# amoretti86/PSVO

Hardware: AMD Instinct MI355X
Metric: particle-steps/sec (higher is better)
Workload: dtype f32

## Files before the change

### psvo_amd/csrc/common.h

```cpp
#pragma once
#include <cstddef>
#include <type_traits>
#include <hip/hip_runtime.h>
#include <stdint.h>

#include "../../include/psvo_hip.h"

#ifndef PSVO_L
#define PSVO_L 1
#endif
#if PSVO_L == 1
#define PSVO_LNS l1
#define PSVO_ENTRY(name) extern "C" int name
#define PSVO_L2_DECL(name) extern "C" __attribute__((visibility("hidden"))) decltype(name) name##_l2;
#elif PSVO_L == 2
#define PSVO_LNS l2
#define PSVO_ENTRY(name) extern "C" __attribute__((visibility("hidden"))) int name##_l2
#define PSVO_L2_DECL(name)
#else
#error "PSVO_L must be 1 or 2"
#endif

namespace psvo {

// ... 434 lines not shown
#pragma unroll
            for (int o = 0; o < DOUT; ++o) gr[o] = lane_fetch(dout[o], src);
            float pre1[NQ][4];
            layer1(w, g, xr, pre1);
            f4v D[NQ];
            hidden2(w, g, r, pre1, D);
            float dp[NQ][4];
#pragma unroll
            for (int jt = 0; jt < NQ; ++jt) {
                float s[4] = {0.f, 0.f, 0.f, 0.f};
#pragma unroll
                for (int o = 0; o < DOUT; ++o) {
                    const float4 wo = *reinterpret_cast<const float4*>(w + kW2 + o * H + 16 * jt + 4 * g);
                    s[0] = fmaf(gr[o], wo.x, s[0]); s[1] = fmaf(gr[o], wo.y, s[1]);
                    s[2] = fmaf(gr[o], wo.z, s[2]); s[3] = fmaf(gr[o], wo.w, s[3]);
                }
#pragma unroll
                for (int v = 0; v < 4; ++v) dp[jt][v] = D[jt][v] > 0.f ? s[v] : 0.f;
            }
            f4v E[NQ];
#pragma unroll
            for (int kt = 0; kt < NQ; ++kt) E[kt] = f4v{0.f, 0.f, 0.f, 0.f};
            const float* wb = w + kWh + 4 * g * kWS + r;
#pragma unroll
            for (int jt = 0; jt < NQ; ++jt) {
#pragma unroll
                for (int v = 0; v < 4; ++v) {
#pragma unroll
                    for (int kt = 0; kt < NQ; ++kt) {
                        const float a = wb[(16 * jt + v) * kWS + 16 * kt];
                        E[kt] = __builtin_amdgcn_mfma_f32_16x16x4f32(a, dp[jt][v], E[kt], 0, 0, 0);
                    }
                }
            }
            float acc[DIN];
#pragma unroll
            for (int d = 0; d < DIN; ++d) acc[d] = 0.f;
#pragma unroll
            for (int q = 0; q < NQ; ++q) {
                float e[4];
#pragma unroll
                for (int c = 0; c < 4; ++c) e[c] = pre1[q][c] > 0.f ? E[q][c] : 0.f;
#pragma unroll
                for (int d = 0; d < DIN; ++d) {
                    const float4 wi = *reinterpret_cast<const float4*>(w + kW1 + d * H + 16 * q + 4 * g);
                    acc[d] = fmaf(e[0], wi.x, fmaf(e[1], wi.y, fmaf(e[2], wi.z, fmaf(e[3], wi.w, acc[d]))));
                }
            }
#pragma unroll
            for (int d = 0; d < DIN; ++d) {
                float v = acc[d];
                v += xor_lane<16>(v);
                v += xor_lane<32>(v);
                const float t = lane_fetch(v, my_row & 15);
                if (mine && (my_row >> 4) == p) dx[d] += t;
            }
        }
    }

    template <bool ROLLED = false>
    __device__ __forceinline__ static void eval(const float* __restrict__ w, const float (&x)[DIN], float (&out)[DOUT]) {
        eval_rows<1, 0>(w, true, x, out);
    }
    template <int S, int PB = 0>
    __device__ __forceinline__ static void eval_part(const float* __restrict__ w, int , const float (&x)[DIN],
                                                     float (&out)[DOUT]) {
        eval_rows<S, PB>(w, true, x, out);
    }
    template <bool ROLLED = false>
    __device__ __forceinline__ static void bwd_input(const float* __restrict__ w, const float (&x)[DIN],
                                                     const float (&dout)[DOUT], float (&dx)[DIN]) {
        bwd_rows<1, 0>(w, x, dout, dx);
    }
    template <int S, int PB = 0>
    __device__ __forceinline__ static void bwd_input_part(const float* __restrict__ w, int , const float (&x)[DIN],
                                                          const float (&dout)[DOUT], float (&dx)[DIN]) {
        bwd_rows<S, PB>(w, x, dout, dx);
    }
};
#endif

template <int D>
__device__ __forceinline__ float diag_lp(const float (&x)[D], const float (&mu)[D], const float (&inv_s)[D],
                                         float cst) {
    float acc = 0.f;
#pragma unroll
    for (int d = 0; d < D; ++d) {
        const float z = (x[d] - mu[d]) * inv_s[d];
        acc = fmaf(z, z, acc);
    }
    return fmaf(-0.5f, acc, cst);
}

template <int CTRL, int ROW_MASK = 0xF, int BANK_MASK = 0xF, bool BOUND = false>
__device__ __forceinline__ float dpp_mov(float old, float v) {
    return __builtin_bit_cast(float, __builtin_amdgcn_update_dpp(__builtin_bit_cast(int, old), __builtin_bit_cast(int, v),
                                                                  CTRL, ROW_MASK, BANK_MASK, BOUND));
}

template <int MASK>
__device__ __forceinline__ float xor_lane(float v) {
    static_assert(MASK == 1 || MASK == 2 || MASK == 4 || MASK == 8 || MASK == 16 || MASK == 32, "xor_lane mask");
    if constexpr (MASK == 1) {
        return dpp_mov<0xB1, 0xF, 0xF, true>(v, v);
    } else if constexpr (MASK == 2) {
        return dpp_mov<0x4E, 0xF, 0xF, true>(v, v);
    } else if constexpr (MASK == 4) {
        float t = dpp_mov<0x104, 0xF, 0x5>(v, v);
        return dpp_mov<0x114, 0xF, 0xA>(t, v);
    } else if constexpr (MASK == 8) {
        return dpp_mov<0x128, 0xF, 0xF, true>(v, v);
    } else if constexpr (MASK == 16) {
        const unsigned u = __builtin_bit_cast(unsigned, v);
        const auto p = __builtin_amdgcn_permlane16_swap(u, u, false, false);
        const bool odd_row = (__lane_id() >> 4) & 1;
        return __builtin_bit_cast(float, odd_row ? p[0] : p[1]);
    } else {
        const unsigned u = __builtin_bit_cast(unsigned, v);
        const auto p = __builtin_amdgcn_permlane32_swap(u, u, false, false);
        return __builtin_bit_cast(float, (__lane_id() >= 32) ? p[0] : p[1]);
    }
}

__device__ __forceinline__ float wave_incl_scan(float v, int ) {
    v += dpp_mov<0x111, 0xF, 0xF, true>(0.f, v);
    v += dpp_mov<0x112, 0xF, 0xF, true>(0.f, v);
    v += dpp_mov<0x114, 0xF, 0xF, true>(0.f, v);
    v += dpp_mov<0x118, 0xF, 0xF, true>(0.f, v);
    v += dpp_mov<0x142, 0xA, 0xF, false>(0.f, v);
    v += dpp_mov<0x143, 0xC, 0xF, false>(0.f, v);
    return v;
}
__device__ __forceinline__ float wave_sum(float v) {
    v = wave_incl_scan(v, 0);
    return __builtin_bit_cast(float, __builtin_amdgcn_readlane(__builtin_bit_cast(int, v), 63));
}
__device__ __forceinline__ float wave_max(float v) {
    const float ninf = -__builtin_huge_valf();
    v = fmaxf(v, dpp_mov<0x111>(ninf, v));
    v = fmaxf(v, dpp_mov<0x112>(ninf, v));
    v = fmaxf(v, dpp_mov<0x114>(ninf, v));
    v = fmaxf(v, dpp_mov<0x118>(ninf, v));
    v = fmaxf(v, dpp_mov<0x142, 0xA>(ninf, v));
    v = fmaxf(v, dpp_mov<0x143, 0xC>(ninf, v));
    return __builtin_bit_cast(float, __builtin_amdgcn_readlane(__builtin_bit_cast(int, v), 63));
}
__device__ __forceinline__ void quad_bcast4(float v, float (&out)[4]) {
    out[0] = dpp_mov<0x00>(v, v);
    out[1] = dpp_mov<0x55>(v, v);
    out[2] = dpp_mov<0xAA>(v, v);
    out[3] = dpp_mov<0xFF>(v, v);
}

template <int G>
__device__ __forceinline__ float group_sum(float v) {
    if constexpr (G > 1) v += xor_lane<1>(v);
    if constexpr (G > 2) v += xor_lane<2>(v);
    if constexpr (G > 4) v += xor_lane<4>(v);
    if constexpr (G > 8) v += xor_lane<8>(v);
    if constexpr (G > 16) v += xor_lane<16>(v);
    if constexpr (G > 32) v += xor_lane<32>(v);
    return v;
}
template <int G>
__device__ __forceinline__ float group_max(float v) {
    if constexpr (G > 1) v = fmaxf(v, xor_lane<1>(v));
    if constexpr (G > 2) v = fmaxf(v, xor_lane<2>(v));
    if constexpr (G > 4) v = fmaxf(v, xor_lane<4>(v));
    if constexpr (G > 8) v = fmaxf(v, xor_lane<8>(v));
    if constexpr (G > 16) v = fmaxf(v, xor_lane<16>(v));
    if constexpr (G > 32) v = fmaxf(v, xor_lane<32>(v));
    return v;
}
template <int G>
__device__ __forceinline__ float group_incl_scan(float v, int m) {
    if constexpr (G > 1) { const float t = dpp_mov<0x111, 0xF, 0xF, true>(0.f, v); v += (m >= 1) ? t : 0.f; }
    if constexpr (G > 2) { const float t = dpp_mov<0x112, 0xF, 0xF, true>(0.f, v); v += (m >= 2) ? t : 0.f; }
    if constexpr (G > 4) { const float t = dpp_mov<0x114, 0xF, 0xF, true>(0.f, v); v += (m >= 4) ? t : 0.f; }
    if constexpr (G > 8) { const float t = dpp_mov<0x118, 0xF, 0xF, true>(0.f, v); v += (m >= 8) ? t : 0.f; }
    if constexpr (G > 16) v += dpp_mov<0x142, 0xA, 0xF, false>(0.f, v);
    if constexpr (G > 32) v += dpp_mov<0x143, 0xC, 0xF, false>(0.f, v);
    return v;
}

__device__ __forceinline__ float lane_bcast(float v, int src) {
    return __builtin_bit_cast(float, __builtin_amdgcn_readlane(__builtin_bit_cast(int, v), src));
}

__device__ __forceinline__ float block_max(float v, float* red, int slot, int wave, int lane, int nw) {
    v = wave_max(v);
    if (nw == 1) return v;
    float* r = red + slot * 16;
    if (lane == 0) r[wave] = v;
    __syncthreads();
    float m = r[0];
    for (int i = 1; i < nw; ++i) m = fmaxf(m, r[i]);
    return m;
}

}
```

### psvo_amd/csrc/filter_bwd.hip

```cpp
#include "common.h"

namespace psvo {
extern int g_tune_deterministic;
inline namespace PSVO_LNS {
PSVO_TIMERS_DEFINE(filter_bwd)


struct FilterBwdArgs {
    int B, T, N;
    int resample, two_q, bootstrap, emission;
    psvo_mlp q1, f, g;
    const float *sig_q1, *sig_q2, *sig_f, *sig_g;
    const float *mu2, *m0, *sig0, *fm0, *fsig0, *obs, *eps;
    const float *X, *Fm, *P1, *logW, *lse;
    const int32_t* idx;
    const float* dlse;
    int nparts;
    const float* dFm_ext;
    const float* dlogW_ext;
    float *dP, *dF, *dG, *dmu2, *dm0, *dfm0;
    float* sacc;
    float* dm2_rows;
    int wave_copies;
    float* scanAB;
// ... 306 lines not shown
        }
        SEC(4);
        MQ::template bwd_input<kRolled>(wq1, x, dPn, dx);
        if (!a.bootstrap) MQ::template bwd_input<kRolled>(wfm, x, dFn, dx);
        SEC(5);

        float dmean1[DX];
#pragma unroll
        for (int d = 0; d < DX; ++d) {
            const float dmu = dx[d];
            inc[AC::kSc + d] += dmu * e[d];
            float dm2 = 0.f;
            if (a.two_q) {
                dmean1[d] = dmu * K.c[d] * K.i1[d];
                dm2 = dmu * K.c[d] * K.i2[d];
                inc[AC::kSmm1 + d] += dmu * mean1[d];
                inc[AC::kSmb + d] += dmu * m2[d];
                inc[AC::kSmm + d] += dmu * mu[d];
                if (valid) a.dm2_rows[(tb * DX + d) * N + n] = dm2;
            } else {
                dmean1[d] = dmu;
            }
        }
        SEC(6);
        if (!first) {
            if constexpr (DET) {
                __syncthreads();
                for (int ph = 0; ph < (nw + nc - 1) / nc; ++ph) {
                    if (ph > 0) __syncthreads();
                    if (valid && wave / nc == ph) {
#pragma unroll
                        for (int d = 0; d < DX; ++d) {
                            if (a.bootstrap) {
                                atomicAdd(&nxtP[d * NT + anc], dmean1[d] + dfmean[d]);
                            } else {
                                atomicAdd(&nxtP[d * NT + anc], dmean1[d]);
                                atomicAdd(&nxtF[d * NT + anc], dfmean[d]);
                            }
                        }
                    }
                }
            } else if (valid) {
#pragma unroll
                for (int d = 0; d < DX; ++d) {
                    if (a.bootstrap) {
                        atomicAdd(&nxtP[d * NT + anc], dmean1[d] + dfmean[d]);
                    } else {
                        atomicAdd(&nxtP[d * NT + anc], dmean1[d]);
                        atomicAdd(&nxtF[d * NT + anc], dfmean[d]);
                    }
                }
            }
        } else {
#pragma unroll
            for (int d = 0; d < DX; ++d) {
                const float s1 = block_sum(dmean1[d], red, wave, lane, nw);
                const float s2 = block_sum(dfmean[d], red, wave, lane, nw);
                if (tid == 0) {
                    const bool same0 = (a.fm0 == a.m0);
                    a.dm0[b * DX + d] = same0 ? s1 + s2 : s1;
                    a.dfm0[b * DX + d] = same0 ? 0.f : s2;
                }
            }
        }
        SEC(7);
        if (t >= 1) {
            c_anc = n_anc;
#pragma unroll
            for (int d = 0; d < DX; ++d) {
                c_x[d] = n_x[d]; c_e[d] = n_e[d]; c_m2[d] = n_m2[d];
                c_mean1[d] = n_mean1[d]; c_fmean[d] = n_fmean[d]; c_dfm[d] = n_dfm[d];
            }
#pragma unroll
            for (int k = 0; k < DY; ++k) c_y[k] = n_y[k];
#pragma unroll
            for (int k = 0; k < 4; ++k) c_sc[k] = n_sc[k];
        }
#pragma unroll
        for (int i = 0; i < AC::kSet; ++i) {
            acc[i] += first ? inc[i] : 0.f;
            acc[AC::kSet + i] += first ? 0.f : inc[i];
        }
        __syncthreads();
        SEC(8);
    }

#pragma unroll
    for (int i = 0; i < AC::kN; ++i) {
        const float s = block_sum(acc[i], red, wave, lane, nw);
        if (tid == 0) a.sacc[(size_t)b * AC::kN + i] = s;
    }
}

template <int DX, int DY, int H>
__global__ void __launch_bounds__(512) filter_bwd_lpp_kernel(const FilterBwdArgs a) {
    using MQ = MlpLds<DX, H, DX, PSVO_L>;
    using MG = MlpLds<DX, H, DY, PSVO_L>;
    using AC = FAcc<DX, DY>;
    constexpr int P = 4;
    extern __shared__ __attribute__((aligned(16))) float smem[];

    const int tid = threadIdx.x, lane = tid & 63, wave = tid >> 6;
    const int NT = blockDim.x, nw = NT >> 6;
    const int NPT = NT / P;
    const int b = blockIdx.x, B = a.B, T = a.T, N = a.N;
    const int pn = tid >> 2, p = tid & 3;
    const bool valid = pn < N;
    const bool one = valid && p == 0;
    const int n = valid ? pn : N - 1;

    float* wq1 = smem;
    float* wf = wq1 + MQ::kSize;
    float* wg = wf + MQ::kSize;
    const int CP = DX * NPT;
    float* accP = wg + MG::kSize;
    float* accF = accP + 2 * nw * CP;
    float* red = accF + 2 * nw * CP;

    MQ::load(wq1, a.q1, tid, NT);
    if (!a.bootstrap) MQ::load(wf, a.f, tid, NT);
    MG::load(wg, a.g, tid, NT);
    const float* wfm = a.bootstrap ? wq1 : wf;
    for (int i = tid; i < 4 * nw * CP; i += NT) accP[i] = 0.f;

    float sq1[DX], sq2[DX], sfv[DX], s0[DX], fs0[DX], isg[DY];
#pragma unroll
    for (int d = 0; d < DX; ++d) {
        sq1[d] = a.sig_q1[d];
        sq2[d] = a.two_q ? a.sig_q2[d] : 1.f;
        sfv[d] = a.bootstrap ? a.sig_q1[d] : a.sig_f[d];
        s0[d] = a.sig0[d];
        fs0[d] = a.fsig0[d];
    }
#pragma unroll
    for (int e = 0; e < DY; ++e) isg[e] = 1.f / a.sig_g[e];
    const BStepK<DX> K0 = make_bstepk<DX>(s0, sq2, fs0, a.two_q != 0);
    const BStepK<DX> K1 = make_bstepk<DX>(sq1, sq2, sfv, a.two_q != 0);

    float acc[AC::kN];
#pragma unroll
    for (int i = 0; i < AC::kN; ++i) acc[i] = 0.f;
    float dlnw = 0.f;

    float m0r[DX], fm0r[DX];
#pragma unroll
    for (int d = 0; d < DX; ++d) {
        m0r[d] = a.m0[b * DX + d];
        fm0r[d] = a.fm0[b * DX + d];
    }
    auto load_anc = [&](int t) -> int {
        return (t >= 1 && a.resample) ? a.idx[((size_t)(t - 1) * B + b) * N + n] : n;
    };
    const bool one_part = (a.nparts == 1);
    auto load_step = [&](int t, int anc, float (&sx)[DX], float (&se)[DX], float (&sm2)[DX], float (&sy)[DY],
                         float (&smean1)[DX], float (&sfmean)[DX], float (&sdfm)[DX], float (&ssc)[4]) {
        const size_t tb = (size_t)t * B + b;
        const size_t tp = (t == 0) ? tb : tb - B;
#pragma unroll
        for (int d = 0; d < DX; ++d) {
            sx[d] = a.X[(tb * DX + d) * N + n];
            se[d] = a.eps[(tb * DX + d) * N + n];
            sm2[d] = a.two_q ? a.mu2[tb * DX + d] : 0.f;
            sfmean[d] = a.Fm[(tp * DX + d) * N + anc];
            smean1[d] = a.bootstrap ? 0.f : a.P1[(tp * DX + d) * N + anc];
            if (a.dFm_ext) {
                if (one_part) {
                    sdfm[d] = a.dFm_ext[(tb * DX + d) * N + n];
                } else {
                    float ext = 0.f;
                    for (int q = 0; q < a.nparts; ++q) ext += a.dFm_ext[((tb * a.nparts + q) * DX + d) * N + n];
                    sdfm[d] = ext;
                }
            } else {
                sdfm[d] = 0.f;
            }
        }
#pragma unroll
        for (int k = 0; k < DY; ++k) sy[k] = a.obs[tb * DY + k];
        ssc[0] = a.logW[tb * N + n];
        ssc[1] = a.lse[tb];
        ssc[2] = a.dlse ? a.dlse[tb] : 0.f;
        if (a.dlogW_ext) {
            if (one_part) {
                ssc[3] = a.dlogW_ext[tb * N + n];
            } else {
                float ext = 0.f;
                for (int q = 0; q < a.nparts; ++q) ext += a.dlogW_ext[(tb * a.nparts + q) * N + n];
                ssc[3] = ext;
            }
        } else {
            ssc[3] = 0.f;
        }
    };
    float c_x[DX], c_e[DX], c_m2[DX], c_y[DY], c_mean1[DX], c_fmean[DX], c_dfm[DX], c_sc[4];
    int c_anc = load_anc(T - 1);
    int anc_next = load_anc(T - 2);
    load_step(T - 1, c_anc, c_x, c_e, c_m2, c_y, c_mean1, c_fmean, c_dfm, c_sc);
    __syncthreads();

    SEC_INIT(filter_bwd)
    auto step = [&](auto first_tag, const int t) {
        SEC(0);
        const size_t tb = (size_t)t * B + b;
        constexpr bool first = decltype(first_tag)::value;
        const BStepK<DX> K = first ? K0 : K1;
        float inc[AC::kSet];
#pragma unroll
        for (int i = 0; i < AC::kSet; ++i) inc[i] = 0.f;
        float* curP = accP + (t & 1) * nw * CP;
        float* nxtP = accP + ((t + 1) & 1) * nw * CP + wave * CP;
        float* curF = accF + (t & 1) * nw * CP;
        float* nxtF = accF + ((t + 1) & 1) * nw * CP + wave * CP;

        float n_x[DX], n_e[DX], n_m2[DX], n_y[DY], n_mean1[DX], n_fmean[DX], n_dfm[DX], n_sc[4];
        int n_anc = n;
        if (t >= 1) {
            n_anc = anc_next;
            load_step(t - 1, n_anc, n_x, n_e, n_m2, n_y, n_mean1, n_fmean, n_dfm, n_sc);
            anc_next = load_anc(t - 2);
        }
        SEC(1);
        float sp[DX], sf[DX];
        {
            float cp[8][DX];
#pragma unroll
            for (int w = 0; w < 8; ++w) {
                const int wc = w < nw ? w : nw - 1;
#pragma unroll
                for (int d = 0; d < DX; ++d) cp[w][d] = curP[wc * CP + d * NPT + pn];
            }
#pragma unroll
            for (int d = 0; d < DX; ++d) {
                sp[d] = 0.f;
#pragma unroll
                for (int w = 0; w < 8; ++w) sp[d] += (w < nw) ? cp[w][d] : 0.f;
                sf[d] = 0.f;
            }
        }
        if (!a.bootstrap) {
            float cf[8][DX];
#pragma unroll
            for (int w = 0; w < 8; ++w) {
                const int wc = w < nw ? w : nw - 1;
#pragma unroll
                for (int d = 0; d < DX; ++d) cf[w][d] = curF[wc * CP + d * NPT + pn];
            }
#pragma unroll
            for (int d = 0; d < DX; ++d)
#pragma unroll
                for (int w = 0; w < 8; ++w) sf[d] += (w < nw) ? cf[w][d] : 0.f;
        }
        float x[DX], e[DX], m2[DX], y[DY], mean1[DX], fmean[DX];
        const int anc = c_anc;
#pragma unroll
        for (int d = 0; d < DX; ++d) {
            x[d] = c_x[d];
            e[d] = c_e[d];
            m2[d] = c_m2[d];
            fmean[d] = first ? fm0r[d] : c_fmean[d];
            mean1[d] = first ? m0r[d] : (a.bootstrap ? c_fmean[d] : c_mean1[d]);
        }
#pragma unroll
        for (int k = 0; k < DY; ++k) y[k] = c_y[k];
        float mu[DX];
#pragma unroll
        for (int d = 0; d < DX; ++d)
            mu[d] = a.two_q ? K.c[d] * fmaf(K.i1[d], mean1[d], K.i2[d] * m2[d]) : mean1[d];

        const float sm = valid ? exp2_fast((c_sc[0] - c_sc[1]) * kLog2e) : 0.f;
        float dlw = c_sc[2] * sm + c_sc[3];
        if (!a.resample) {
            const float tot = block_sum(one ? dlnw : 0.f, red, wave, lane, nw);
            dlw += dlnw - sm * tot;
        }
        if (!valid) dlw = 0.f;
        dlnw = first ? 0.f : dlw;
        const float cnt = (p == 0) ? 1.f : 0.f;

        SEC(2);
        float dxp[DX];
#pragma unroll
        for (int d = 0; d < DX; ++d) dxp[d] = 0.f;
        {
            float gm[DY], dgm[DY];
            MG::template eval_part<P>(wg, p, x, gm);
#pragma unroll
            for (int k = 0; k < DY; ++k) {
                gm[k] = group_sum<P>(gm[k]);
                float dmean = 1.f;
                if (a.emission) { dmean = emis_dmean(gm[k]); gm[k] = emis_mean(gm[k]); }
                const float z = (y[k] - gm[k]) * isg[k];
                dgm[k] = dlw * z * isg[k] * dmean;
                acc[AC::kSg + k] += cnt * dlw * (z * z - 1.f) * isg[k];
                if (valid && p == 2) a.dG[(tb * DY + k) * N + n] = dgm[k];
            }
            MG::template bwd_input_part<P>(wg, p, x, dgm, dxp);
        }
        SEC(3);
        float dfmean[DX];
#pragma unroll
        for (int d = 0; d < DX; ++d) {
            const float z = (x[d] - fmean[d]) * K.ifs[d];
            const float tf = dlw * z * K.ifs[d];
            dxp[d] -= cnt * tf;
            dfmean[d] = tf;
            inc[AC::kSfs + d] += dlw * (z * z - 1.f) * K.ifs[d];
            inc[AC::kSc + d] += dlw * K.ic[d];
        }
        float dPn[DX], dFn[DX];
#pragma unroll
        for (int d = 0; d < DX; ++d) {
            dPn[d] = sp[d];
            const float ext = c_dfm[d];
            if (a.bootstrap) {
                dPn[d] += ext;
                dFn[d] = 0.f;
            } else {
                dFn[d] = sf[d] + ext;
            }
            if (!valid) {
                dPn[d] = 0.f;
                dFn[d] = 0.f;
            }
        }
        for (int w = p; w < nw; w += 4) {
#pragma unroll
            for (int d = 0; d < DX; ++d) {
                curP[w * CP + d * NPT + pn] = 0.f;
                if (!a.bootstrap) curF[w * CP + d * NPT + pn] = 0.f;
            }
        }
        if (valid) {
            if (p == 0) {
#pragma unroll
                for (int d = 0; d < DX; ++d) a.dP[(tb * DX + d) * N + n] = dPn[d];
            } else if (p == 1 && !a.bootstrap) {
#pragma unroll
                for (int d = 0; d < DX; ++d) a.dF[(tb * DX + d) * N + n] = dFn[d];
            }
        }
        SEC(4);
        MQ::template bwd_input_part<P>(wq1, p, x, dPn, dxp);
        if (!a.bootstrap) MQ::template bwd_input_part<P>(wfm, p, x, dFn, dxp);
        SEC(5);

        float dmean1[DX];
#pragma unroll
        for (int d = 0; d < DX; ++d) {
            const float dmu = group_sum<P>(dxp[d]);
            inc[AC::kSc + d] += dmu * e[d];
            if (a.two_q) {
                dmean1[d] = dmu * K.c[d] * K.i1[d];
                const float dm2 = dmu * K.c[d] * K.i2[d];
                inc[AC::kSmm1 + d] += dmu * mean1[d];
                inc[AC::kSmb + d] += dmu * m2[d];
                inc[AC::kSmm + d] += dmu * mu[d];
                if (valid && p == 3) a.dm2_rows[(tb * DX + d) * N + n] = dm2;
            } else {
                dmean1[d] = dmu;
            }
        }
        SEC(6);
        if (!first) {
            if (valid) {
#pragma unroll
                for (int d = 0; d < DX; ++d) {
                    if ((d & 3) == p) {
                        if (a.bootstrap) {
                            atomicAdd(&nxtP[d * NPT + anc], dmean1[d] + dfmean[d]);
                        } else {
                            atomicAdd(&nxtP[d * NPT + anc], dmean1[d]);
                            atomicAdd(&nxtF[d * NPT + anc], dfmean[d]);
                        }
                    }
                }
            }
        } else {
#pragma unroll
            for (int d = 0; d < DX; ++d) {
                const float s1 = block_sum(one ? dmean1[d] : 0.f, red, wave, lane, nw);
                const float s2 = block_sum(one ? dfmean[d] : 0.f, red, wave, lane, nw);
                if (tid == 0) {
                    const bool same0 = (a.fm0 == a.m0);
                    a.dm0[b * DX + d] = same0 ? s1 + s2 : s1;
                    a.dfm0[b * DX + d] = same0 ? 0.f : s2;
                }
            }
        }
        SEC(7);
        if (t >= 1) {
            c_anc = n_anc;
#pragma unroll
            for (int d = 0; d < DX; ++d) {
                c_x[d] = n_x[d]; c_e[d] = n_e[d]; c_m2[d] = n_m2[d];
                c_mean1[d] = n_mean1[d]; c_fmean[d] = n_fmean[d]; c_dfm[d] = n_dfm[d];
            }
#pragma unroll
            for (int k = 0; k < DY; ++k) c_y[k] = n_y[k];
#pragma unroll
            for (int k = 0; k < 4; ++k) c_sc[k] = n_sc[k];
        }
#pragma unroll
        for (int i = 0; i < AC::kSet; ++i) {
            acc[i] += (first && p == 0) ? inc[i] : 0.f;
            acc[AC::kSet + i] += (!first && p == 0) ? inc[i] : 0.f;
        }
        __syncthreads();
        SEC(8);
    };
    for (int t = T - 1; t >= 1; --t) step(std::false_type{}, t);
    step(std::true_type{}, 0);

#pragma unroll
    for (int i = 0; i < AC::kN; ++i) {
        const float s = block_sum(valid ? acc[i] : 0.f, red, wave, lane, nw);
        if (tid == 0) a.sacc[(size_t)b * AC::kN + i] = s;
    }
}

template <int DX, int DY>
__global__ void filter_bwd_finalize(const float* __restrict__ sacc, int B, int two_q, int bootstrap,
                                    const float* sig_q1, const float* sig_q2, const float* sig0, int same0,
                                    float* dsig_q1, float* dsig_q2, float* dsig_f, float* dsig_g, float* dsig0,
                                    float* dfsig0) {
    using AC = FAcc<DX, DY>;
    const int d = threadIdx.x;
    if (d < DX) {
        float S[2 * AC::kSet];
        for (int i = 0; i < 2 * AC::kSet; ++i) S[i] = 0.f;
        for (int b = 0; b < B; ++b)
            for (int i = 0; i < 2 * AC::kSet; ++i) S[i] += sacc[(size_t)b * AC::kN + i];
        float ds2 = 0.f;
        for (int set = 0; set < 2; ++set) {
            const float* P = S + set * AC::kSet;
            const float s1 = set ? sig_q1[d] : sig0[d];
            float ds1;
            if (two_q) {
                const float i1 = 1.f / s1, i2 = 1.f / sig_q2[d];
                const float c = 1.f / (i1 + i2);
                const float dc = P[AC::kSc + d] + P[AC::kSmm + d] / c;
                const float di1 = c * P[AC::kSmm1 + d] - c * c * dc;
                const float di2 = c * P[AC::kSmb + d] - c * c * dc;
                ds1 = -i1 * i1 * di1;
                ds2 += -i2 * i2 * di2;
            } else {
                ds1 = P[AC::kSc + d];
            }
            const float dfs = P[AC::kSfs + d];
            if (set) {
                dsig_q1[d] = ds1 + (bootstrap ? dfs : 0.f);
                dsig_f[d] = bootstrap ? 0.f : dfs;
            } else {
                dsig0[d] = same0 ? ds1 + dfs : ds1;
                dfsig0[d] = same0 ? 0.f : dfs;
            }
        }
        dsig_q2[d] = ds2;
    }
    if (d < DY) {
        float s = 0.f;
        for (int b = 0; b < B; ++b) s += sacc[(size_t)b * AC::kN + AC::kSg + d];
        dsig_g[d] = s;
    }
}

__global__ void __launch_bounds__(256) row_sum_kernel(const float* __restrict__ in, long long rows, int L,
                                                      float* __restrict__ out) {
    const long long r = (long long)blockIdx.x * 4 + (threadIdx.x >> 6);
    if (r >= rows) return;
    const int lane = threadIdx.x & 63;
    float s = 0.f;
    for (int l = lane; l < L; l += 64) s += in[r * L + l];
    s = wave_sum(s);
    if (lane == 0) out[r] = s;
}

#if PSVO_L == 1
template <int DX>
struct ScanRec {
    static constexpr int NC = DX * DX + DX;
    static constexpr int kExt = NC, kAnc = NC + DX;
    static constexpr int REC = scan_rec_floats(DX);
};

template <int DX, int DY, int H>
__global__ void __launch_bounds__(512) fbs_coeff_kernel(const FilterBwdArgs a) {
    using MQ = MlpLds<DX, H, DX, 1>;
    using MG = MlpLds<DX, H, DY, 1>;
    using SR = ScanRec<DX>;
    constexpr bool kRolled = true;
    extern __shared__ __attribute__((aligned(16))) float smem[];
    const int tid = threadIdx.x, NT = blockDim.x;
    const int t = blockIdx.x, b = blockIdx.y, B = a.B, N = a.N;
    const bool valid = tid < N;
    const int n = valid ? tid : N - 1;
    const size_t tb = (size_t)t * B + b;
    float rec[SR::REC];
#pragma unroll
    for (int i = 0; i < SR::REC; ++i) rec[i] = 0.f;
#pragma unroll
    for (int d = 0; d < DX; ++d) rec[SR::kExt + d] = a.dFm_ext ? a.dFm_ext[(tb * DX + d) * N + n] : 0.f;
    if (t >= 1) {
        float* wq1 = smem;
        float* wg = wq1 + MQ::kSize;
        MQ::load(wq1, a.q1, tid, NT);
        MG::load(wg, a.g, tid, NT);
        float x[DX], fmean[DX], y[DY];
        const int anc = a.idx[(tb - B) * N + n];
        rec[SR::kAnc] = __int_as_float(anc);
#pragma unroll
        for (int d = 0; d < DX; ++d) {
            x[d] = a.X[(tb * DX + d) * N + n];
            fmean[d] = a.Fm[((tb - B) * DX + d) * N + anc];
        }
#pragma unroll
        for (int k = 0; k < DY; ++k) y[k] = a.obs[tb * DY + k];
        const float sm = exp2_fast((a.logW[tb * N + n] - a.lse[tb]) * kLog2e);
        const float dlw = (a.dlse ? a.dlse[tb] : 0.f) * sm + (a.dlogW_ext ? a.dlogW_ext[tb * N + n] : 0.f);
        float kap[DX], ifs[DX];
#pragma unroll
        for (int d = 0; d < DX; ++d) {
            const float i1 = 1.f / a.sig_q1[d];
            kap[d] = a.two_q ? i1 / (i1 + 1.f / a.sig_q2[d]) : 1.f;
            ifs[d] = i1;
        }
        __syncthreads();
        float dxg[DX];
#pragma unroll
        for (int d = 0; d < DX; ++d) dxg[d] = 0.f;
        {
            float gm[DY], dgm[DY];
            MG::template eval<kRolled>(wg, x, gm);
#pragma unroll
            for (int k = 0; k < DY; ++k) {
                float dmean = 1.f;
                if (a.emission) { dmean = emis_dmean(gm[k]); gm[k] = emis_mean(gm[k]); }
                const float isg = 1.f / a.sig_g[k];
                dgm[k] = dlw * (y[k] - gm[k]) * isg * isg * dmean;
            }
            MG::template bwd_input<kRolled>(wg, x, dgm, dxg);
        }
#pragma unroll
        for (int d = 0; d < DX; ++d) {
            const float tf = dlw * (x[d] - fmean[d]) * ifs[d] * ifs[d];
            rec[DX * DX + d] = fmaf(kap[d], dxg[d] - tf, tf);
        }
#pragma unroll
        for (int k = 0; k < DX; ++k) {
            float ek[DX], col[DX];
#pragma unroll
            for (int d = 0; d < DX; ++d) { ek[d] = (d == k) ? 1.f : 0.f; col[d] = 0.f; }
            MQ::template bwd_input<kRolled>(wq1, x, ek, col);
#pragma unroll
// ... 376 lines not shown
```

### psvo_amd/csrc/filter_fwd.hip

```cpp
#include "common.h"

namespace psvo {
inline namespace PSVO_LNS {
PSVO_TIMERS_DEFINE(filter_fwd)


struct FilterArgs {
    int B, T, N;
    int resample, two_q, bootstrap, emission;
    psvo_mlp q1, f, g;
    const float *sig_q1, *sig_q2, *sig_f, *sig_g;
    const float *mu2, *m0, *sig0, *fm0, *fsig0, *obs, *eps, *u;
    const int32_t* idx_in;
    float *X, *Xanc, *Fm, *P1, *logW;
    int32_t* idx_out;
    float* lse;
};

template <int DX>
struct StepK {
    float c[DX];
    float ic[DX];
    float i1[DX];
    float i2[DX];
// ... 158 lines not shown
            }
            a.logW[tb * N + n] = lw;
        }

        SEC(4);
        const float mx = block_max(lw, red, 0, wave, lane, nw);
        const float w = valid ? exp2_fast((lw - mx) * kLog2e) : 0.f;
        float sc = wave_incl_scan(w, lane);
        float total;
        if (nw > 1) {
            float* wt = red + 32;
            if (lane == 63) wt[wave] = sc;
            __syncthreads();
            float off = 0.f, tot = 0.f;
            for (int i = 0; i < nw; ++i) {
                const float v = wt[i];
                if (i < wave) off += v;
                tot += v;
            }
            sc += off;
            total = tot;
        } else {
            total = lane_bcast(sc, 63);
        }
        const float lse_t = fmaf(kLn2, log2_fast(total), mx);
        if (tid == 0) a.lse[tb] = lse_t;

        SEC(5);
        if (a.resample) {
            cdf[tid] = sc;
#pragma unroll
            for (int d = 0; d < DX; ++d) {
                sx[d * NT + tid] = x[d];
                sp[d * NT + tid] = p1[d];
                if (!a.bootstrap) sf[d * NT + tid] = fm[d];
            }
            __syncthreads();
            SEC(6);
            int idx;
            if (a.idx_in) {
                idx = idx_c;
            } else {
                const float target = u_c * total;
                int pos = 0;
                for (int s = 1 << (31 - __clz(N)); s > 0; s >>= 1) {
                    const int p = pos + s;
                    if (p <= N && cdf[p - 1] <= target) pos = p;
                }
                idx = min(pos, N - 1);
            }
#pragma unroll
            for (int d = 0; d < DX; ++d) {
                x[d] = sx[d * NT + idx];
                mean1[d] = sp[d * NT + idx];
                fmean[d] = a.bootstrap ? mean1[d] : sf[d * NT + idx];
            }
            if (valid) {
                a.idx_out[tb * N + n] = idx;
#pragma unroll
                for (int d = 0; d < DX; ++d) a.Xanc[(tb * DX + d) * N + n] = x[d];
            }
            lnw = neg_logN;
            SEC(7);
            __syncthreads();
        } else {
#pragma unroll
            for (int d = 0; d < DX; ++d) {
                mean1[d] = p1[d];
                fmean[d] = fm[d];
            }
            if (valid) {
                a.idx_out[tb * N + n] = n;
#pragma unroll
                for (int d = 0; d < DX; ++d) a.Xanc[(tb * DX + d) * N + n] = x[d];
            }
            lnw = lw - lse_t;
            if (nw > 1) __syncthreads();
        }

#pragma unroll
        for (int d = 0; d < DX; ++d) {
            eps_c[d] = eps_n[d];
            mu2_c[d] = mu2_n[d];
        }
#pragma unroll
        for (int k = 0; k < DY; ++k) obs_c[k] = obs_n[k];
        u_c = u_n;
        idx_c = idx_n;
    }
}

template <int DX, int DY, int H, int MAXT>
__global__ void __launch_bounds__(MAXT) filter_fwd_lpp_kernel(const FilterArgs a) {
    using MQ = MlpLds<DX, H, DX, PSVO_L>;
    using MG = MlpLds<DX, H, DY, PSVO_L>;
    constexpr int P = 4;
    constexpr bool kOpaque = false;
    extern __shared__ __attribute__((aligned(16))) float smem[];

    const int tid = threadIdx.x, lane = tid & 63, wave = tid >> 6;
    const int NT = blockDim.x, nw = NT >> 6;
    const int NPT = NT / P;
    const int b = blockIdx.x, B = a.B, T = a.T, N = a.N;
    const int pn = tid >> 2, p = tid & 3;
    const int uwave = __builtin_amdgcn_readfirstlane(wave);
    const bool valid = pn < N;
    const int n = valid ? pn : N - 1;

    float* wq1 = smem;
    float* wf = wq1 + MQ::kSize;
    float* wg = wf + MQ::kSize;
    float* cdf = wg + MG::kSize;
    float* piv = cdf + NPT;
    float* sx = piv + 16;
    float* sp = sx + DX * NPT;
    float* sf = sp + DX * NPT;
    float* red = sf + DX * NPT;

    MQ::load(wq1, a.q1, tid, NT);
    if (!a.bootstrap) MQ::load(wf, a.f, tid, NT);
    MG::load(wg, a.g, tid, NT);
    const float* wfm = a.bootstrap ? wq1 : wf;
    if (tid < 16) piv[tid] = __builtin_huge_valf();

    float sq1[DX], sq2[DX], sfv[DX], s0[DX], fs0[DX], isg[DY];
    float lg = -DY * kHalfLog2Pi;
#pragma unroll
    for (int d = 0; d < DX; ++d) {
        sq1[d] = a.sig_q1[d];
        sq2[d] = a.two_q ? a.sig_q2[d] : 1.f;
        sfv[d] = a.bootstrap ? a.sig_q1[d] : a.sig_f[d];
        s0[d] = a.sig0[d];
        fs0[d] = a.fsig0[d];
    }
#pragma unroll
    for (int e = 0; e < DY; ++e) {
        const float s = a.sig_g[e];
        isg[e] = 1.f / s;
        lg -= logf(s);
    }
    const StepK<DX> K0 = make_stepk<DX>(s0, sq2, fs0, a.two_q != 0);
    const StepK<DX> K1 = make_stepk<DX>(sq1, sq2, sfv, a.two_q != 0);
    const float neg_logN = -logf((float)N);
    const float ninf = -__builtin_huge_valf();

    float mean1[DX], fmean[DX];
#pragma unroll
    for (int d = 0; d < DX; ++d) {
        mean1[d] = a.m0[b * DX + d];
        fmean[d] = a.fm0[b * DX + d];
    }
    float lnw = neg_logN;

    float eps_c[DX], mu2_c[DX], obs_c[DY], u_c = 0.f;
    int idx_c = 0;
    auto load_inputs = [&](int t, float (&e)[DX], float (&m)[DX], float (&o)[DY], float& uu, int& ii) {
        const size_t tb = (size_t)t * B + b;
#pragma unroll
        for (int d = 0; d < DX; ++d) {
            e[d] = a.eps[(tb * DX + d) * N + n];
            m[d] = a.two_q ? a.mu2[tb * DX + d] : 0.f;
        }
#pragma unroll
        for (int k = 0; k < DY; ++k) o[k] = a.obs[tb * DY + k];
        if (a.resample) {
            if (a.idx_in) ii = a.idx_in[tb * N + n];
            else uu = a.u[tb * N + n];
        }
    };
    load_inputs(0, eps_c, mu2_c, obs_c, u_c, idx_c);
    __syncthreads();

    SEC_INIT(filter_fwd)
    auto step = [&](auto first_tag, const int t) {
        SEC(0);
        const size_t tb = (size_t)t * B + b;
        const StepK<DX> K = decltype(first_tag)::value ? K0 : K1;
        float eps_n[DX], mu2_n[DX], obs_n[DY], u_n = 0.f;
        int idx_n = 0;
        if (t + 1 < T) load_inputs(t + 1, eps_n, mu2_n, obs_n, u_n, idx_n);

        SEC(1);
        float mu[DX], x[DX];
#pragma unroll
        for (int d = 0; d < DX; ++d) {
            mu[d] = a.two_q ? K.c[d] * fmaf(K.i1[d], mean1[d], K.i2[d] * mu2_c[d]) : mean1[d];
            x[d] = fmaf(K.c[d], eps_c[d], mu[d]);
        }
        const float q_lp = diag_lp<DX>(x, mu, K.ic, K.lq);
        const float f_lp = diag_lp<DX>(x, fmean, K.ifs, K.lf);

        SEC(2);
        int zo = 0;
        if (kOpaque) asm volatile("" : "+v"(zo));
        float gm[DY], p1[DX], fm[DX];
        MG::template eval_part<P>(wg + zo, p, x, gm);
        MQ::template eval_part<P>(wq1 + zo, p, x, p1);
        if (!a.bootstrap) MQ::template eval_part<P>(wfm + zo, p, x, fm);
#pragma unroll
        for (int k = 0; k < DY; ++k) gm[k] = group_sum<P>(gm[k]);
        if (a.emission) {
#pragma unroll
            for (int k = 0; k < DY; ++k) gm[k] = emis_mean(gm[k]);
        }
#pragma unroll
        for (int d = 0; d < DX; ++d) {
            p1[d] = group_sum<P>(p1[d]);
            fm[d] = a.bootstrap ? p1[d] : group_sum<P>(fm[d]);
        }
        const float g_lp = diag_lp<DY>(obs_c, gm, isg, lg);
        float lw = f_lp + g_lp - q_lp + lnw;
        if (!valid) lw = ninf;

        if (valid) {
            if (p == 0) {
#pragma unroll
                for (int d = 0; d < DX; ++d) a.X[(tb * DX + d) * N + n] = x[d];
                a.logW[tb * N + n] = lw;
            } else if (p == 1) {
#pragma unroll
                for (int d = 0; d < DX; ++d) a.Fm[(tb * DX + d) * N + n] = fm[d];
            } else if (p == 2 && a.P1) {
#pragma unroll
                for (int d = 0; d < DX; ++d) a.P1[(tb * DX + d) * N + n] = p1[d];
            }
        }

        SEC(3);
        const float wmx = wave_max(lw);
        const float wbase = (wmx == ninf) ? 0.f : wmx;
        const float w = (valid && p == 0) ? exp2_fast((lw - wbase) * kLog2e) : 0.f;
        float sc = wave_incl_scan(w, lane);
        if (lane == 63) {
            red[wave] = wmx;
            red[16 + wave] = sc;
        }
        if (a.resample) {
            if (p == 1) {
#pragma unroll
                for (int d = 0; d < DX; ++d) sx[d * NPT + pn] = x[d];
            } else if (p == 2) {
#pragma unroll
                for (int d = 0; d < DX; ++d) sp[d * NPT + pn] = p1[d];
            } else if (p == 3 && !a.bootstrap) {
#pragma unroll
                for (int d = 0; d < DX; ++d) sf[d * NPT + pn] = fm[d];
            }
        }
        SEC(4);
        __syncthreads();
        SEC(5);
        const int li = lane & 15;
        const float m_i = li < nw ? red[li] : ninf;
        const float s_i = li < nw ? red[16 + li] : 0.f;
        const float gmx = lane_bcast(group_max<16>(m_i), 0);
        const float gbase = (gmx == ninf) ? 0.f : gmx;
        const float v_i = s_i * exp2_fast((m_i - gbase) * kLog2e);
        const float pre = group_incl_scan<16>(v_i, li);
        const float total = lane_bcast(pre, nw - 1);
        const float off = uwave > 0 ? lane_bcast(pre, max(uwave - 1, 0)) : 0.f;
        sc = fmaf(sc, exp2_fast((wbase - gbase) * kLog2e), off);
        const float lse_t = fmaf(kLn2, log2_fast(total), gmx);
        if (tid == 3) a.lse[tb] = lse_t;

        SEC(6);
        if (a.resample) {
            if (p == 0) {
                cdf[pn] = sc;
                if ((pn & 15) == 15) piv[pn >> 4] = sc;
            }
            __syncthreads();
            SEC(7);
            int idx;
            if (a.idx_in) {
                idx = idx_c;
            } else {
                const float target = u_c * total;
                const float4 pv = *reinterpret_cast<const float4*>(piv + 4 * p);
                float c1 = (pv.x <= target ? 1.f : 0.f) + (pv.y <= target ? 1.f : 0.f) +
                           (pv.z <= target ? 1.f : 0.f) + (pv.w <= target ? 1.f : 0.f);
                c1 = group_sum<P>(c1);
                const int blk = min((int)c1, (NPT >> 4) - 1);
                const float4 cv = *reinterpret_cast<const float4*>(cdf + 16 * blk + 4 * p);
                float c2 = (cv.x <= target ? 1.f : 0.f) + (cv.y <= target ? 1.f : 0.f) +
                           (cv.z <= target ? 1.f : 0.f) + (cv.w <= target ? 1.f : 0.f);
                c2 = group_sum<P>(c2);
                idx = min(16 * blk + (int)c2, N - 1);
            }
#pragma unroll
            for (int d = 0; d < DX; ++d) {
                x[d] = sx[d * NPT + idx];
                mean1[d] = sp[d * NPT + idx];
                fmean[d] = a.bootstrap ? mean1[d] : sf[d * NPT + idx];
            }
            if (valid) {
                if (p == 3) a.idx_out[tb * N + n] = idx;
                if (p == 0) {
#pragma unroll
                    for (int d = 0; d < DX; ++d) a.Xanc[(tb * DX + d) * N + n] = x[d];
                }
            }
            lnw = neg_logN;
            SEC(8);
            __syncthreads();
            SEC(9);
        } else {
#pragma unroll
            for (int d = 0; d < DX; ++d) {
                mean1[d] = p1[d];
                fmean[d] = fm[d];
            }
            if (valid) {
                if (p == 3) a.idx_out[tb * N + n] = n;
                if (p == 0) {
#pragma unroll
                    for (int d = 0; d < DX; ++d) a.Xanc[(tb * DX + d) * N + n] = x[d];
                }
            }
            lnw = lw - lse_t;
            __syncthreads();
        }

#pragma unroll
        for (int d = 0; d < DX; ++d) {
            eps_c[d] = eps_n[d];
            mu2_c[d] = mu2_n[d];
        }
#pragma unroll
        for (int k = 0; k < DY; ++k) obs_c[k] = obs_n[k];
        u_c = u_n;
        idx_c = idx_n;
    };
    step(std::true_type{}, 0);
    for (int t = 1; t < T; ++t) step(std::false_type{}, t);
}

template <int DX, int DY, int H>
static int launch_filter(const FilterArgs& a, hipStream_t stream) {
    using MQ = MlpLds<DX, H, DX, PSVO_L>;
    using MG = MlpLds<DX, H, DY, PSVO_L>;
    constexpr bool kLppOk = (H % 16 == 0) && (PSVO_L == 2 || (H <= 32 && DX <= 3) || H == 16);
    if constexpr (kLppOk) {
        if (a.N <= 128) {
            const int NT4 = (4 * a.N + 63) & ~63;
            const int NPT = NT4 / 4;
            const size_t lds4 = sizeof(float) * (2 * MQ::kSize + MG::kSize + NPT + 16 + 3 * DX * NPT + 32);
            clear_hip_error();
            hipLaunchKernelGGL((filter_fwd_lpp_kernel<DX, DY, H, 512>), dim3(a.B), dim3(NT4), lds4, stream, a);
            return launch_status();
        }
    }
    const int NT = (a.N + 63) & ~63;
    const size_t lds = sizeof(float) * (2 * MQ::kSize + MG::kSize + NT + 3 * DX * NT + 48);
    clear_hip_error();
    if (NT <= 256 && a.emission)
        hipLaunchKernelGGL((filter_fwd_kernel<DX, DY, H, 256, 1>), dim3(a.B), dim3(NT), lds, stream, a);
    else if (NT <= 256)
        hipLaunchKernelGGL((filter_fwd_kernel<DX, DY, H, 256, 0>), dim3(a.B), dim3(NT), lds, stream, a);
    else
        hipLaunchKernelGGL((filter_fwd_kernel<DX, DY, H, 512>), dim3(a.B), dim3(NT), lds, stream, a);
    return launch_status();
}

}
}

PSVO_L2_DECL(psvo_filter_forward)
PSVO_ENTRY(psvo_filter_forward)(const psvo_desc* desc, const psvo_mlp* q1, const psvo_mlp* f, const psvo_mlp* g,
                                   const float* sig_q1, const float* sig_q2, const float* sig_f,
                                   const float* sig_g, const float* mu2, const float* m0, const float* sig0,
                                   const float* fm0, const float* fsig0, const float* obs, const float* eps,
                                   const float* u, const int32_t* idx_in, float* X, float* Xanc, float* Fm, float* P1,
                                   float* logW, int32_t* idx_out, float* lse, void* stream) {
    using namespace psvo;
    if (!desc_layers_ok(desc)) return PSVO_ERR_UNSUPPORTED;
#if PSVO_L == 1
    if (desc && desc->layers == 2)
        return psvo_filter_forward_l2(desc, q1, f, g, sig_q1, sig_q2, sig_f, sig_g, mu2, m0, sig0, fm0, fsig0, obs,
            eps, u, idx_in, X, Xanc, Fm, P1, logW, idx_out, lse, stream);
#endif
    if (!mlp_layers_ok(q1) || !mlp_layers_ok(f) || !mlp_layers_ok(g)) return PSVO_ERR_INVALID;
    if (!desc || !q1 || !g || !sig_q1 || !sig_g || !m0 || !sig0 || !fm0 || !fsig0 || !obs || !eps || !X ||
        !Xanc || !Fm || !logW || !idx_out || !lse)
        return PSVO_ERR_INVALID;
    if (desc->B <= 0 || desc->T <= 0 || desc->N <= 0) return PSVO_ERR_INVALID;
    if (desc->two_q && (!mu2 || !sig_q2)) return PSVO_ERR_INVALID;
    if (!desc->bootstrap && (!f || !sig_f)) return PSVO_ERR_INVALID;
    if (desc->resample && !u && !idx_in) return PSVO_ERR_INVALID;
    if (desc->N > 512) return PSVO_ERR_UNSUPPORTED;

    FilterArgs a;
    a.B = desc->B; a.T = desc->T; a.N = desc->N;
    a.resample = desc->resample; a.two_q = desc->two_q; a.bootstrap = desc->bootstrap; a.emission = desc->emission;
    a.q1 = *q1; a.f = desc->bootstrap ? *q1 : *f; a.g = *g;
    a.sig_q1 = sig_q1; a.sig_q2 = sig_q2; a.sig_f = sig_f; a.sig_g = sig_g;
    a.mu2 = mu2; a.m0 = m0; a.sig0 = sig0; a.fm0 = fm0; a.fsig0 = fsig0;
    a.obs = obs; a.eps = eps; a.u = u; a.idx_in = idx_in;
    a.X = X; a.Xanc = Xanc; a.Fm = Fm; a.P1 = P1; a.logW = logW; a.idx_out = idx_out; a.lse = lse;
    hipStream_t s = static_cast<hipStream_t>(stream);
    return dispatch_shape(desc->Dx, desc->Dy, desc->H, [&](auto dx, auto dy, auto h) {
        return launch_filter<dx(), dy(), h()>(a, s); });
}
```

Baseline: 241.5 million.

## Distribute per-step input loads across quad lanes and broadcast via DPP

Each particle is handled by a quad of lanes (indexed by p). Instead of every lane loading every per-step input field (eps, X, Fm, P1, mu2, obs, logW, lse, ancestor index, etc.), the fields are packed into slots so that each lane loads only one field per slot. The values are then broadcast within the quad using DPP quad permutes. Per-field pointers and strides are precomputed once and decremented or incremented each step, replacing index arithmetic. This cuts redundant global loads and VGPRs in both the forward and backward filter kernels, at the cost of extra DPP moves, a switch-based field select, and more complex pointer bookkeeping, including the lagged ancestor and gather handling in the backward pass.

After: 248.7 million (median of 6 runs). 1.03x the previous value.

```diff
diff --git a/psvo_amd/csrc/common.h b/psvo_amd/csrc/common.h
--- a/psvo_amd/csrc/common.h
+++ b/psvo_amd/csrc/common.h
@@ -610,6 +610,19 @@
     out[3] = dpp_mov<0xFF>(v, v);
 }
 
+typedef float __attribute__((__may_alias__)) in_word_t;
+
+template <int NS>
+__device__ __forceinline__ float quad_field(const float (&slot)[NS], int f) {
+    const float v = slot[f >> 2];
+    switch (f & 3) {
+        case 0: return dpp_mov<0x00>(v, v);
+        case 1: return dpp_mov<0x55>(v, v);
+        case 2: return dpp_mov<0xAA>(v, v);
+        default: return dpp_mov<0xFF>(v, v);
+    }
+}
+
 template <int G>
 __device__ __forceinline__ float group_sum(float v) {
     if constexpr (G > 1) v += xor_lane<1>(v);
diff --git a/psvo_amd/csrc/filter_bwd.hip b/psvo_amd/csrc/filter_bwd.hip
--- a/psvo_amd/csrc/filter_bwd.hip
+++ b/psvo_amd/csrc/filter_bwd.hip
@@ -482,50 +482,115 @@
         return (t >= 1 && a.resample) ? a.idx[((size_t)(t - 1) * B + b) * N + n] : n;
     };
     const bool one_part = (a.nparts == 1);
-    auto load_step = [&](int t, int anc, float (&sx)[DX], float (&se)[DX], float (&sm2)[DX], float (&sy)[DY],
-                         float (&smean1)[DX], float (&sfmean)[DX], float (&sdfm)[DX], float (&ssc)[4]) {
+    const bool ext_fm = a.dFm_ext && one_part, ext_lw = a.dlogW_ext && one_part;
+    constexpr int kFX = 0, kFE = DX, kFFm = 2 * DX, kFDf = 3 * DX, kFLw = 4 * DX, kFDlw = 4 * DX + 1, kFAnc = 4 * DX + 2,
+                  kFM2 = 4 * DX + 3, kFY = 5 * DX + 3, kFLse = 5 * DX + 3 + DY, kFDlse = kFLse + 1, kFP1 = kFLse + 2,
+                  kFields = kFP1 + DX, kSlots = (kFields + 3) / 4;
+    static_assert(kFAnc >= kFFm + DX && kFAnc < kFP1, "the ancestor field (lag 2) lies outside the gathered (lag 1) ranges");
+    const int nslots = a.bootstrap ? (kFP1 + 3) / 4 : kSlots;
+    auto slot_gathers = [](int s) { return (4 * s < kFFm + DX && 4 * s + 3 >= kFFm) || (4 * s < kFP1 + DX && 4 * s + 3 >= kFP1); };
+    auto slot_lags = [&](int s) { return slot_gathers(s) || (4 * s <= kFAnc && 4 * s + 3 >= kFAnc); };
+    const in_word_t* in_ptr[kSlots];
+    int in_str[kSlots], in_lag[kSlots];
+    auto field_ptr = [&](int f, const in_word_t*& ptr, int& str, int& lg) {
+        const in_word_t* q = nullptr;
+        int w = 0, lag = 0;
+        if (f < kFE) { q = a.X + (size_t)(b * DX + f - kFX) * N + n; w = DX * N; }
+        else if (f < kFFm) { q = a.eps + (size_t)(b * DX + f - kFE) * N + n; w = DX * N; }
+        else if (f < kFDf) { q = a.Fm + (size_t)(b * DX + f - kFFm) * N; w = DX * N; lag = 1; }
+        else if (f < kFLw) { if (ext_fm) { q = a.dFm_ext + (size_t)(b * DX + f - kFDf) * N + n; w = DX * N; } }
+        else if (f == kFLw) { q = a.logW + (size_t)b * N + n; w = N; }
+        else if (f == kFDlw) { if (ext_lw) { q = a.dlogW_ext + (size_t)b * N + n; w = N; } }
+        else if (f == kFAnc) { if (a.resample) { q = reinterpret_cast<const in_word_t*>(a.idx) + (size_t)b * N + n; w = N; lag = 2; } }
+        else if (f < kFY) { if (a.two_q) { q = a.mu2 + b * DX + f - kFM2; w = DX; } }
+        else if (f < kFLse) { q = a.obs + b * DY + f - kFY; w = DY; }
+        else if (f == kFLse) { q = a.lse + b; w = 1; }
+        else if (f == kFDlse) { if (a.dlse) { q = a.dlse + b; w = 1; } }
+        else if (f < kFields) { if (!a.bootstrap) { q = a.P1 + (size_t)(b * DX + f - kFP1) * N; w = DX * N; lag = 1; } }
+        if (q) {
+            ptr = q + (size_t)max(T - 1 - lag, 0) * B * w;
+            str = B * w;
+            lg = lag;
+        } else {
+            ptr = a.eps + (size_t)b * DX * N + n;
+            str = 0;
+            lg = 0;
+        }
+    };
+#pragma unroll
+    for (int s = 0; s < kSlots; ++s) {
+        field_ptr(4 * s, in_ptr[s], in_str[s], in_lag[s]);
+#pragma unroll
+        for (int j = 1; j < 4; ++j) {
+            const in_word_t* q;
+            int st, lg;
+            field_ptr(4 * s + j, q, st, lg);
+            in_ptr[s] = (p == j) ? q : in_ptr[s];
+            in_str[s] = (p == j) ? st : in_str[s];
+            in_lag[s] = (p == j) ? lg : in_lag[s];
+        }
+    }
+    float raw_n[kSlots];
+#pragma unroll
+    for (int s = 0; s < kSlots; ++s) raw_n[s] = 0.f;
+    auto issue_step = [&](int t, int anc) {
+#pragma unroll
+        for (int s = 0; s < kSlots; ++s) {
+            if (s < nslots) {
+                if (slot_gathers(s)) raw_n[s] = in_ptr[s][in_lag[s] == 1 ? anc : 0];
+                else raw_n[s] = *in_ptr[s];
+                if (slot_lags(s)) in_ptr[s] -= (t > in_lag[s]) ? in_str[s] : 0;
+                else in_ptr[s] -= in_str[s];
+            }
+        }
+    };
+    auto issue_parts = [&](int t, float (&sdfm)[DX], float& sdlw) {
         const size_t tb = (size_t)t * B + b;
-        const size_t tp = (t == 0) ? tb : tb - B;
-#pragma unroll
-        for (int d = 0; d < DX; ++d) {
-            sx[d] = a.X[(tb * DX + d) * N + n];
-            se[d] = a.eps[(tb * DX + d) * N + n];
-            sm2[d] = a.two_q ? a.mu2[tb * DX + d] : 0.f;
-            sfmean[d] = a.Fm[(tp * DX + d) * N + anc];
-            smean1[d] = a.bootstrap ? 0.f : a.P1[(tp * DX + d) * N + anc];
-            if (a.dFm_ext) {
-                if (one_part) {
-                    sdfm[d] = a.dFm_ext[(tb * DX + d) * N + n];
-                } else {
-                    float ext = 0.f;
-                    for (int q = 0; q < a.nparts; ++q) ext += a.dFm_ext[((tb * a.nparts + q) * DX + d) * N + n];
-                    sdfm[d] = ext;
-                }
-            } else {
-                sdfm[d] = 0.f;
-            }
-        }
-#pragma unroll
-        for (int k = 0; k < DY; ++k) sy[k] = a.obs[tb * DY + k];
-        ssc[0] = a.logW[tb * N + n];
-        ssc[1] = a.lse[tb];
-        ssc[2] = a.dlse ? a.dlse[tb] : 0.f;
-        if (a.dlogW_ext) {
-            if (one_part) {
-                ssc[3] = a.dlogW_ext[tb * N + n];
-            } else {
+        if (a.dFm_ext && !one_part) {
+#pragma unroll
+            for (int d = 0; d < DX; ++d) {
                 float ext = 0.f;
-                for (int q = 0; q < a.nparts; ++q) ext += a.dlogW_ext[(tb * a.nparts + q) * N + n];
-                ssc[3] = ext;
-            }
-        } else {
-            ssc[3] = 0.f;
+                for (int q = 0; q < a.nparts; ++q) ext += a.dFm_ext[((tb * a.nparts + q) * DX + d) * N + n];
+                sdfm[d] = ext;
+            }
+        }
+        if (a.dlogW_ext && !one_part) {
+            float ext = 0.f;
+            for (int q = 0; q < a.nparts; ++q) ext += a.dlogW_ext[(tb * a.nparts + q) * N + n];
+            sdlw = ext;
         }
     };
     float c_x[DX], c_e[DX], c_m2[DX], c_y[DY], c_mean1[DX], c_fmean[DX], c_dfm[DX], c_sc[4];
-    int c_anc = load_anc(T - 1);
-    int anc_next = load_anc(T - 2);
-    load_step(T - 1, c_anc, c_x, c_e, c_m2, c_y, c_mean1, c_fmean, c_dfm, c_sc);
+    int c_anc = load_anc(T - 1), anc_next = n;
+    auto take_step = [&](int t, const float (&pdfm)[DX], float pdlw) {
+#pragma unroll
+        for (int d = 0; d < DX; ++d) {
+            c_x[d] = quad_field(raw_n, kFX + d);
+            c_e[d] = quad_field(raw_n, kFE + d);
+            const float m2 = quad_field(raw_n, kFM2 + d), p1 = quad_field(raw_n, kFP1 + d), df = quad_field(raw_n, kFDf + d);
+            c_m2[d] = a.two_q ? m2 : 0.f;
+            c_fmean[d] = quad_field(raw_n, kFFm + d);
+            c_mean1[d] = a.bootstrap ? 0.f : p1;
+            c_dfm[d] = a.dFm_ext ? (one_part ? df : pdfm[d]) : 0.f;
+        }
+#pragma unroll
+        for (int k = 0; k < DY; ++k) c_y[k] = quad_field(raw_n, kFY + k);
+        const float dlse = quad_field(raw_n, kFDlse), dlw = quad_field(raw_n, kFDlw);
+        const int an = __builtin_bit_cast(int, quad_field(raw_n, kFAnc));
+        c_sc[0] = quad_field(raw_n, kFLw);
+        c_sc[1] = quad_field(raw_n, kFLse);
+        c_sc[2] = a.dlse ? dlse : 0.f;
+        c_sc[3] = a.dlogW_ext ? (one_part ? dlw : pdlw) : 0.f;
+        anc_next = (a.resample && t >= 2) ? an : n;
+    };
+    {
+        float pdfm[DX], pdlw = 0.f;
+#pragma unroll
+        for (int d = 0; d < DX; ++d) pdfm[d] = 0.f;
+        issue_step(T - 1, c_anc);
+        issue_parts(T - 1, pdfm, pdlw);
+        take_step(T - 1, pdfm, pdlw);
+    }
     __syncthreads();
 
     SEC_INIT(filter_bwd)
@@ -542,12 +607,13 @@
         float* curF = accF + (t & 1) * nw * CP;
         float* nxtF = accF + ((t + 1) & 1) * nw * CP + wave * CP;
 
-        float n_x[DX], n_e[DX], n_m2[DX], n_y[DY], n_mean1[DX], n_fmean[DX], n_dfm[DX], n_sc[4];
-        int n_anc = n;
+        float n_dfm[DX], n_dlw = 0.f;
+#pragma unroll
+        for (int d = 0; d < DX; ++d) n_dfm[d] = 0.f;
+        const int n_anc = anc_next;
         if (t >= 1) {
-            n_anc = anc_next;
-            load_step(t - 1, n_anc, n_x, n_e, n_m2, n_y, n_mean1, n_fmean, n_dfm, n_sc);
-            anc_next = load_anc(t - 2);
+            issue_step(t - 1, n_anc);
+            issue_parts(t - 1, n_dfm, n_dlw);
         }
         SEC(1);
         float sp[DX], sf[DX];
@@ -720,15 +786,7 @@
         SEC(7);
         if (t >= 1) {
             c_anc = n_anc;
-#pragma unroll
-            for (int d = 0; d < DX; ++d) {
-                c_x[d] = n_x[d]; c_e[d] = n_e[d]; c_m2[d] = n_m2[d];
-                c_mean1[d] = n_mean1[d]; c_fmean[d] = n_fmean[d]; c_dfm[d] = n_dfm[d];
-            }
-#pragma unroll
-            for (int k = 0; k < DY; ++k) c_y[k] = n_y[k];
-#pragma unroll
-            for (int k = 0; k < 4; ++k) c_sc[k] = n_sc[k];
+            take_step(t - 1, n_dfm, n_dlw);
         }
 #pragma unroll
         for (int i = 0; i < AC::kSet; ++i) {
diff --git a/psvo_amd/csrc/filter_fwd.hip b/psvo_amd/csrc/filter_fwd.hip
--- a/psvo_amd/csrc/filter_fwd.hip
+++ b/psvo_amd/csrc/filter_fwd.hip
@@ -334,23 +334,66 @@
     }
     float lnw = neg_logN;
 
+    constexpr int kFU = DX, kFM2 = DX + 1, kFY = 2 * DX + 1, kFields = 2 * DX + 1 + DY, kSlots = (kFields + 3) / 4;
+    const in_word_t* in_ptr[kSlots];
+    int in_str[kSlots];
+    auto field_ptr = [&](int f, const in_word_t*& q, int& st) {
+        q = a.eps + (size_t)b * DX * N + n;
+        st = 0;
+        if (f < kFU) {
+            q = a.eps + ((size_t)b * DX + f) * N + n;
+            st = B * DX * N;
+        } else if (f == kFU) {
+            if (a.resample) {
+                q = (a.idx_in ? reinterpret_cast<const in_word_t*>(a.idx_in) : static_cast<const in_word_t*>(a.u)) + (size_t)b * N + n;
+                st = B * N;
+            }
+        } else if (f < kFY) {
+            if (a.two_q) {
+                q = a.mu2 + (size_t)b * DX + (f - kFM2);
+                st = B * DX;
+            }
+        } else if (f < kFields) {
+            q = a.obs + (size_t)b * DY + (f - kFY);
+            st = B * DY;
+        }
+    };
+#pragma unroll
+    for (int s = 0; s < kSlots; ++s) {
+        field_ptr(4 * s, in_ptr[s], in_str[s]);
+#pragma unroll
+        for (int j = 1; j < 4; ++j) {
+            const in_word_t* q;
+            int st;
+            field_ptr(4 * s + j, q, st);
+            in_ptr[s] = (p == j) ? q : in_ptr[s];
+            in_str[s] = (p == j) ? st : in_str[s];
+        }
+    }
     float eps_c[DX], mu2_c[DX], obs_c[DY], u_c = 0.f;
     int idx_c = 0;
-    auto load_inputs = [&](int t, float (&e)[DX], float (&m)[DX], float (&o)[DY], float& uu, int& ii) {
-        const size_t tb = (size_t)t * B + b;
+    float raw_n[kSlots];
+    auto issue_inputs = [&]() {
+#pragma unroll
+        for (int s = 0; s < kSlots; ++s) {
+            raw_n[s] = *in_ptr[s];
+            in_ptr[s] += in_str[s];
+        }
+    };
+    auto take_inputs = [&]() {
 #pragma unroll
         for (int d = 0; d < DX; ++d) {
-            e[d] = a.eps[(tb * DX + d) * N + n];
-            m[d] = a.two_q ? a.mu2[tb * DX + d] : 0.f;
-        }
-#pragma unroll
-        for (int k = 0; k < DY; ++k) o[k] = a.obs[tb * DY + k];
-        if (a.resample) {
-            if (a.idx_in) ii = a.idx_in[tb * N + n];
-            else uu = a.u[tb * N + n];
-        }
+            eps_c[d] = quad_field(raw_n, d);
+            const float m = quad_field(raw_n, kFM2 + d);
+            mu2_c[d] = a.two_q ? m : 0.f;
+        }
+#pragma unroll
+        for (int k = 0; k < DY; ++k) obs_c[k] = quad_field(raw_n, kFY + k);
+        u_c = quad_field(raw_n, kFU);
+        idx_c = __builtin_bit_cast(int, u_c);
     };
-    load_inputs(0, eps_c, mu2_c, obs_c, u_c, idx_c);
+    issue_inputs();
+    take_inputs();
     __syncthreads();
 
     SEC_INIT(filter_fwd)
@@ -358,9 +401,7 @@
         SEC(0);
         const size_t tb = (size_t)t * B + b;
         const StepK<DX> K = decltype(first_tag)::value ? K0 : K1;
-        float eps_n[DX], mu2_n[DX], obs_n[DY], u_n = 0.f;
-        int idx_n = 0;
-        if (t + 1 < T) load_inputs(t + 1, eps_n, mu2_n, obs_n, u_n, idx_n);
+        if (t + 1 < T) issue_inputs();
 
         SEC(1);
         float mu[DX], x[DX];
@@ -503,15 +544,7 @@
             __syncthreads();
         }
 
-#pragma unroll
-        for (int d = 0; d < DX; ++d) {
-            eps_c[d] = eps_n[d];
-            mu2_c[d] = mu2_n[d];
-        }
-#pragma unroll
-        for (int k = 0; k < DY; ++k) obs_c[k] = obs_n[k];
-        u_c = u_n;
-        idx_c = idx_n;
+        take_inputs();
     };
     step(std::true_type{}, 0);
     for (int t = 1; t < T; ++t) step(std::false_type{}, t);
```
